# CEED/Laghos

Measured on AMD Instinct MI355X. Metric: Mdofs×steps/s on 3D Sedov -pa (Q3/Q2), higher is better.
Workload: dtype f64; 1 GPU; 3D Sedov -p 1 -m cube01_hex -rs 4 -ok 3 -ot 2 -pa (32^3 elements, E0/2^dim = 0.125); transport=none (one rank), elements=32768, h1_dofs=2738019, l2_dofs=884736, quad_points_per_element=216, rk_stages_executed=1300, ode=RK4, parallelism=elements1x1x1, zones_per_gpu=32x32x32

## Files before the change

laghos_amd/csrc/lgh_api.hip:

```cpp
#include <cstdarg>
#include <cstdlib>
#include <cmath>
#include <algorithm>
#include <limits>

#include "lgh_common.hpp"

#include <atomic>
#include <chrono>
#include <dlfcn.h>

namespace lgh
{

static thread_local char g_err[512] = "";
void set_error(const char *fmt, ...)
{
   va_list ap;
   va_start(ap, fmt);
   vsnprintf(g_err, sizeof(g_err), fmt, ap);
   va_end(ap);
}

__global__ void __launch_bounds__(256) vec_set_k(double *y, double a, long n)
{
   for (long i = blockIdx.x * (long)blockDim.x + threadIdx.x; i < n; i += (long)gridDim.x * blockDim.x) { y[i] = a; }
}
__global__ void __launch_bounds__(256)
vec_axpby_k(double *z, double a, const double *x, double b, const double *y, long n)
{
   for (long i = blockIdx.x * (long)blockDim.x + threadIdx.x; i < n; i += (long)gridDim.x * blockDim.x)
   {
      z[i] = fma(a, x[i], __dmul_rn(b, y[i]));
   }
}
__global__ void __launch_bounds__(256)
vec_axpby2_k(double2 *z, double a, const double2 *x, double b, const double2 *y, long n2)
{
   const long stride = (long)gridDim.x * blockDim.x;
   long i = blockIdx.x * (long)blockDim.x + threadIdx.x;
   for (; i + stride < n2; i += 2 * stride)
   {
      const double2 x0 = x[i], y0 = y[i], x1 = x[i + stride], y1 = y[i + stride];
      z[i] = make_double2(fma(a, x0.x, __dmul_rn(b, y0.x)), fma(a, x0.y, __dmul_rn(b, y0.y)));
      z[i + stride] = make_double2(fma(a, x1.x, __dmul_rn(b, y1.x)), fma(a, x1.y, __dmul_rn(b, y1.y)));
   }
   if (i < n2)
   {
      const double2 x0 = x[i], y0 = y[i];
      z[i] = make_double2(fma(a, x0.x, __dmul_rn(b, y0.x)), fma(a, x0.y, __dmul_rn(b, y0.y)));
   }
}
__global__ void __launch_bounds__(256)
vec_axpby_pair_k(double2 *z1, double a1, const double2 *x1, double b1, double2 *z2, double a2, const double2 *x2, double b2, const double2 *y, long n2)
{
   const long stride = (long)gridDim.x * blockDim.x;
   for (long i = blockIdx.x * (long)blockDim.x + threadIdx.x; i < n2; i += stride)
   {
      const double2 y0 = y[i], p = x1[i], q = x2[i];
// ... 28 lines not shown
   }
}
__global__ void set_double_k(double *p, double v) { *p = v; }
__global__ void __launch_bounds__(256) dt_est_set_k(double *p, double v)
{
   if (threadIdx.x == 0) { p[0] = v; }
   for (int s = threadIdx.x; s < kDtSlots; s += blockDim.x) { p[kDtSlotStride * (1 + s)] = __builtin_inf(); }
}
__global__ void __launch_bounds__(256) dt_est_fold_k(double *p, const int *err, double *host_out, const unsigned long long token)
{
   __shared__ double red[16];
   double m = __builtin_inf();
   for (int s = threadIdx.x; s < kDtSlots; s += blockDim.x)
   {
      m = fmin(m, p[kDtSlotStride * (1 + s)]);
      p[kDtSlotStride * (1 + s)] = __builtin_inf();
   }
   m = block_min(m, red);
   if (threadIdx.x == 0)
   {
      const double est = fmin(p[0], m);
      p[0] = est;
      host_out[0] = est;
      ((int *)(host_out + 1))[0] = *err;
      __threadfence_system();
      __hip_atomic_store((unsigned long long *)(host_out + 2), token, __ATOMIC_RELEASE, __HIP_MEMORY_SCOPE_SYSTEM);
   }
}

int vec_set(lgh_ctx *c, double *y, double a, long n)
{
   if (n <= 0) { return LGH_OK; }
   hipLaunchKernelGGL(vec_set_k, dim3(grid_for(n)), dim3(256), 0, c->stream, y, a, n);
   LGH_HIP_CHECK(hipGetLastError());
   return LGH_OK;
}
int vec_axpby(lgh_ctx *c, double *z, double a, const double *x, double b, const double *y, long n)
{
   if (n <= 0) { return LGH_OK; }
   if (n >= 4096 && (((uintptr_t)z | (uintptr_t)x | (uintptr_t)y) & 15u) == 0)
   {
      const long n2 = n / 2;
      hipLaunchKernelGGL(vec_axpby2_k, dim3(grid_for(n2)), dim3(256), 0, c->stream, (double2 *)z, a, (const double2 *)x, b,
                         (const double2 *)y, n2);
      if (n & 1) { hipLaunchKernelGGL(vec_axpby_k, dim3(1), dim3(64), 0, c->stream, z + 2 * n2, a, x + 2 * n2, b, y + 2 * n2, 1L); }
   }
   else { hipLaunchKernelGGL(vec_axpby_k, dim3(grid_for(n)), dim3(256), 0, c->stream, z, a, x, b, y, n); }
   LGH_HIP_CHECK(hipGetLastError());
   return LGH_OK;
}
int vec_axpby_pair(lgh_ctx *c, double *z1, double a1, const double *x1, double b1, double *z2, double a2, const double *x2, double b2,
                   const double *y, long n)
{
   if (n <= 0) { return LGH_OK; }
   if (n >= 4096 && (((uintptr_t)z1 | (uintptr_t)x1 | (uintptr_t)z2 | (uintptr_t)x2 | (uintptr_t)y) & 15u) == 0)
   {
      const long n2 = n / 2;
      hipLaunchKernelGGL(vec_axpby_pair_k, dim3(grid_for(n2)), dim3(256), 0, c->stream, (double2 *)z1, a1, (const double2 *)x1, b1, (double2 *)z2, a2,
                         (const double2 *)x2, b2, (const double2 *)y, n2);
      LGH_HIP_CHECK(hipGetLastError());
      if (n & 1)
      {
         hipLaunchKernelGGL(vec_axpby_k, dim3(1), dim3(64), 0, c->stream, z1 + 2 * n2, a1, x1 + 2 * n2, b1, y + 2 * n2, 1L);
         hipLaunchKernelGGL(vec_axpby_k, dim3(1), dim3(64), 0, c->stream, z2 + 2 * n2, a2, x2 + 2 * n2, b2, y + 2 * n2, 1L);
      }
      LGH_HIP_CHECK(hipGetLastError());
// ... 527 lines not shown
   LGH_CHECK_ARG(c && on);
   *on = (!c->stress_store && c->erhs_q && c->force_e_q && c->v_snap && !c->fused_forces_off && c->dim == 3) ? 0 : 1;
   return LGH_OK;
}
int lgh_qupdate_store_stress(lgh_ctx *c, int on)
{
   LGH_CHECK_ARG(c);
   if ((on != 0) != (c->stress_store != 0))
   {
      c->stress_store = on ? 1 : 0;
      invalidate_fused(c);
      c->stress_current = 0;
   }
   return LGH_OK;
}
int lgh_reset_quadrature_data(lgh_ctx *c)
{
   LGH_CHECK_ARG(c);
   invalidate_fused(c);
   return LGH_OK;
}
int lgh_fused_force_mult(lgh_ctx *c, double *y_h1)
{
   LGH_CHECK_ARG(c && y_h1);
   if (!(c->force_e_q && c->fused_f1_valid)) { set_error("lgh_fused_force_mult: no fused F.1 on hand"); return LGH_ERR_ARG; }
   int rc = h1_transpose_gather(c, c->dim, c->force_e_q, y_h1);
   if (rc == LGH_OK && c->multi != 0) { rc = halo_sum(c, y_h1, c->dim); }
   return rc;
}
int lgh_fused_force_mult_transpose(lgh_ctx *c, double *y_l2)
{
   LGH_CHECK_ARG(c && y_l2);
   if (!(c->erhs_q && c->fused_ftv_valid)) { set_error("lgh_fused_force_mult_transpose: no fused F^T v on hand"); return LGH_ERR_ARG; }
   LGH_HIP_CHECK(hipMemcpyAsync(y_l2, c->erhs_q, sizeof(double) * (size_t)c->L2V, hipMemcpyDeviceToDevice, c->stream));
   return LGH_OK;
}
int lgh_quadrature_generation(lgh_ctx *c, unsigned long *gen, int *f1_valid, int *ftv_valid)
{
   LGH_CHECK_ARG(c && gen && f1_valid && ftv_valid);
   *gen = c->qgen;
   *f1_valid = c->fused_f1_valid;
   *ftv_valid = c->fused_ftv_valid;
   return LGH_OK;
}
double *lgh_qdata_Jac0inv(lgh_ctx *c) { return c->Jac0inv; }
double *lgh_qdata_rho0DetJ0w(lgh_ctx *c) { return c->rho0DetJ0w; }
double *lgh_mass_D(lgh_ctx *c)
{
   c->mass_rank1 = -1;
   c->mass_gen++;
   return c->massD;
}
int lgh_mass_data_form(lgh_ctx *c, int *form)
{
   LGH_CHECK_ARG(c && form);
   if (c->dim == 1) { *form = 0; return LGH_OK; }
   const double *Dq, *Se;
   int dqs;
   int rc = mass_data(c, &Dq, &dqs, &Se);
   if (rc) { return rc; }
   *form = (c->mass_rank1 == 1) ? 1 : 0;
   return LGH_OK;
}
int lgh_mass_data_changed(lgh_ctx *c)
{
   LGH_CHECK_ARG(c);
   c->mass_rank1 = -1;
   c->mass_gen++;
// ... 252 lines not shown
         for (int cc = 0; cc < dim; cc++)
         {
            c->timers.c[0] += its[cc];
            if (h1_iters) { *h1_iters += its[cc]; }
         }
         c->cur_ess = dim - 1;
         return LGH_OK;
      }
      if (rc != LGH_ERR_UNSUPPORTED) { return rc; }
   }
   for (int cc = 0; cc < dim; cc++)
   {
      LGH_HIP_CHECK(hipMemcpyAsync(work_B, rhs_h1 + (size_t)cc * N, sizeof(double) * N,
                                   hipMemcpyDeviceToDevice, c->stream));
      rc = lgh_mass_set_essential_tdofs(c, cc);
      if (rc) { return rc; }
      rc = lgh_mass_eliminate_rhs(c, work_B);
      if (rc) { return rc; }
      int it = 0;
      timer_start(c);
      rc = cg_solve(c, LGH_SPACE_H1, work_B, dv + (size_t)cc * N, rel_tol, max_iter, &it, true);
      timer_stop(c, 0);
      if (rc) { return rc; }
      c->timers.c[0] += it;
      if (h1_iters) { *h1_iters += it; }
   }
   return LGH_OK;
}

int lgh_vec_set(lgh_ctx *c, double *y, double a, long n) { LGH_CHECK_ARG(c && y); return vec_set(c, y, a, n); }
int lgh_vec_copy(lgh_ctx *c, double *y, const double *x, long n)
{
   LGH_CHECK_ARG(c && y && x);
   LGH_HIP_CHECK(hipMemcpyAsync(y, x, sizeof(double) * n, hipMemcpyDeviceToDevice, c->stream));
   return LGH_OK;
}
int lgh_vec_axpby(lgh_ctx *c, double *z, double a, const double *x, double b, const double *y, long n)
{
   LGH_CHECK_ARG(c && z && x && y);
   return vec_axpby(c, z, a, x, b, y, n);
}
int lgh_vec_axpby_pair(lgh_ctx *c, double *z1, double a1, const double *x1, double b1, double *z2, double a2, const double *x2, double b2,
                       const double *y, long n)
{
   LGH_CHECK_ARG(c && z1 && x1 && z2 && x2 && y && n >= 0);
   {
      auto overlap = [n](const double *p, const double *q) { return p < q + n && q < p + n; };
      LGH_CHECK_ARG(!overlap(z1, z2) && !overlap(z1, x2) && !overlap(z1, y));
      LGH_CHECK_ARG(!overlap(z2, y) && !overlap(z2, x1) && (z2 == x2 || !overlap(z2, x2)) && (z1 == x1 || !overlap(z1, x1)));
   }
   return vec_axpby_pair(c, z1, a1, x1, b1, z2, a2, x2, b2, y, n);
}
int lgh_vec_dot(lgh_ctx *c, const double *x, const double *y, long n, double *result)
{
   LGH_CHECK_ARG(c && x && y && result);
   int rc = vec_dot(c, x, y, nullptr, n, c->scal + 1);
   if (rc) { return rc; }
   LGH_HIP_CHECK(hipMemcpyAsync(c->host_pinned + kPinDot, c->scal + 1, sizeof(double), hipMemcpyDeviceToHost, c->stream));
   LGH_HIP_CHECK(hipStreamSynchronize(c->stream));
   *result = c->host_pinned[kPinDot];
   return LGH_OK;
}

int lgh_set_velocity_source(lgh_ctx *c, const double *accel_h1)
{
   LGH_CHECK_ARG(c);
   if (accel_h1)
   {
// ... 213 lines not shown
```

laghos_amd/csrc/lgh_common.hpp:

```cpp
#pragma once
#include <hip/hip_runtime.h>

#include <algorithm>
#include <cstdint>
#include <cstdio>
#include <cstring>
#include <string>
#include <vector>

#include "../../include/laghos_hip.h"

namespace lgh
{

void set_error(const char *fmt, ...);

#define LGH_HIP_CHECK(expr)                                                              \
   do                                                                                    \
   {                                                                                     \
      hipError_t e_ = (expr);                                                            \
      if (e_ != hipSuccess)                                                              \
      {                                                                                  \
         lgh::set_error("HIP error %s at %s:%d: %s", hipGetErrorName(e_), __FILE__,      \
                        __LINE__, #expr);                                                \
// ... 147 lines not shown
   lgh::ScalarCg *l2run = nullptr;
   const double *accel_src;
   lgh::EnergySolve energy;
   long ls_stats[3] = {0, 0, 0};
   bool own_stream;

   double *B, *G, *Bl, *W, *gamma;
   int *h1map;
   int *t_off;
   int *t_idx;
   int *t_ell;
   int t_deg;
   uint8_t *essmask[3];
   int *ess[3];
   int ess_count[3];
   double *owner;
   int cur_ess;

   double *stressJinvT, *Jac0inv, *rho0DetJ0w, *massD, *diagV, *dinvV;
   double *Jac0inv_soa;
   double *Jac0inv_e;
   int jac0_compact;
   double *massS, *ones_ne;
   double *M1h = nullptr, *M1l = nullptr;
   double *w1d = nullptr;
   int mass_rank1;
   double *dt_est_dev;
   double *erhs_q;
   double *v_snap;
   double *force_e_q;
   int fused_ftv_valid, fused_f1_valid;
   unsigned long qgen;
   int *dev_flags;
   double *ones_l2;
   int stress_store;
   int stress_current;
   int fused_forces_off;
   double *XE;
   double *YE;
   double *cg_r, *cg_z, *cg_d0, *cg_d1, *cg_y;
   double *partials;
   int part_stride;
   unsigned int *tickets;
   lgh::CgScalars *cgs;
   double *scal;
   double *host_pinned;
   unsigned long long look_token;
   double *host_pinned_dev;

   void *vcg_s;
   double *vcg_vec, *vcg_partials;
   unsigned int *vcg_tickets;
   unsigned vcg_stride;
   int vcg_last;
   int vcg_grid;
   int b_h1_sym, b_l2_sym;
   int ncu;
   void *vcg_aux;

   lgh::Timers timers;
   lgh::KTime *ktime;
   int cg_last_iters[2][3];
   lgh::Comm *comm;
   int nranks, rank;
   int multi;
   unsigned long long *q_trace_dev;
// ... 243 lines not shown
int vcg_test_exact_sum(lgh_ctx *c, int mode, long n, int G, int E, const double *scale, const double *v, const long long *w_in,
                       long long *w_out, double *d_out, int *i_out);
int vcg_k1_form(lgh_ctx *c);
void comm_shared_nodes(const lgh_ctx *c, const uint8_t **hmask, const int **sh_node, int *n_shared);
int energy_overlap_poll(lgh_ctx *c);
int host_wait_token(lgh_ctx *c, volatile unsigned long long *word, unsigned long long token);
constexpr int kLsWord = 50;
constexpr int kLsWordsPerSet = 56;
struct LockstepWords { const long long *own; const long long *peers; int n_peers, before; };
bool l2_lockstep_possible(lgh_ctx *c);
int cg_l2_begin_lockstep(lgh_ctx *c, const double *b, double *x, double rel_tol, int max_iter);
int l2_lockstep_limit(lgh_ctx *c);
int l2_lockstep_apply(lgh_ctx *c, int it, const LockstepWords &prev, double *den_mirror);
int l2_lockstep_update(lgh_ctx *c, int it, const double *den_src, long long *word_out);
int l2_lockstep_fold(lgh_ctx *c, int it, const LockstepWords &last);
int cg_l2_end_lockstep(lgh_ctx *c, int *iters);
int comm_ranks_before(const lgh_ctx *c);
bool vcg_lockstep_ready(const lgh_ctx *c);
int cg_l2_begin(lgh_ctx *c, const double *b, double *x, double rel_tol, int max_iter);
int cg_l2_end(lgh_ctx *c, int *iters);
void cg_l2_free(lgh_ctx *c);
int cg_solve(lgh_ctx *c, int space, const double *b, double *x, double rel_tol, int max_iter,
             int *iters, bool x_is_zero);
int stress_on_hand(lgh_ctx *c, const char *who);
int qupdate(lgh_ctx *c, const double *S);
int setup_rho0detj0(lgh_ctx *c, const double *x0, const double *rho0_l2, const double *rho0_q,
                    double *volume);
int interp_energy(lgh_ctx *c, int which, const double *vec, double *result);
int tg_source_2d(lgh_ctx *c, const double *S, double *out);
int test_eig(lgh_ctx *c, int dim, int n, const double *A, double *lambda, double *vec);
int test_singular(lgh_ctx *c, int dim, int n, const double *A, double *sv);
int test_sqrt(lgh_ctx *c, int n, const double *x, double *y);
int vec_set(lgh_ctx *c, double *y, double a, long n);
int vec_axpby(lgh_ctx *c, double *z, double a, const double *x, double b, const double *y, long n);
int vec_axpby_pair(lgh_ctx *c, double *z1, double a1, const double *x1, double b1, double *z2, double a2, const double *x2, double b2,
                   const double *y, long n);
int vec_neg_inplace(lgh_ctx *c, double *y, long n);
int vec_zero_list(lgh_ctx *c, double *y, const int *list, int n);
int vec_dot(lgh_ctx *c, const double *x, const double *y, const double *w, long n, double *dev_out);
struct HaloNodeAlias { const int *nodes, *sh_node; };
int halo_sum(lgh_ctx *c, double *v, int ncomp, double *extra = nullptr, int nextra = 0, bool packed = false, const HaloNodeAlias *alias = nullptr);
void comm_node_lists(const lgh_ctx *c, const int **nodes, int *total, const int **sh_node, int *n_shared);
struct HaloPackTables
{
   const int *sh_off, *sh_src;
   const int *pos, *cnt;
   const int *base, *ncnt;
   double *sbuf;
   int n_nbr;
};
bool comm_pack_tables(const lgh_ctx *c, HaloPackTables *t);
bool halo_can_piggyback(const lgh_ctx *c);
bool comm_second_channel(const lgh_ctx *c);
int exchange_words(lgh_ctx *c, const long long *src, int nwords);
int comm_word_peers(lgh_ctx *c, int nwords, const long long **peers, int *n_peers);
int allreduce_dev_n(lgh_ctx *c, double *dev, long count, int op);
int allreduce_dev(lgh_ctx *c, double *dev, int count, int op, bool packed = false);

bool kernel_id_supported_1d(int kid);
int create_1d(const lgh_config *cfg, lgh_ctx *c);
int setup_1d(lgh_ctx *c, const double *x0, const double *rho0_l2, const double *rho0_q, double *volume);
int mass_changed_1d(lgh_ctx *c);
int force_mult_1d(lgh_ctx *c, const double *x_l2, double *y_h1);
int force_mult_t_1d(lgh_ctx *c, const double *v_h1, double *y_l2);
int mass_apply_1d(lgh_ctx *c, int space, const double *x, double *y, bool eliminate);
int l2_solve_local_1d(lgh_ctx *c, const double *b, double *x);
// ... 44 lines not shown
```

laghos_amd/csrc/lgh_energy.hip:

```cpp
#include <algorithm>

#include "lgh_common.hpp"

extern "C"
{

__global__ void __launch_bounds__(256) vec_differs_k(const double *__restrict__ a, const double *__restrict__ b, const long n, int *flag)
{
   const long stride = (long)gridDim.x * blockDim.x, t = (long)blockIdx.x * blockDim.x + threadIdx.x;
   bool diff = false;
   if (((((uintptr_t)a) | ((uintptr_t)b)) & 15u) == 0)
   {
      const longlong2 *a2 = (const longlong2 *)a, *b2 = (const longlong2 *)b;
      for (long i = t; i < n / 2; i += stride)
      {
         const longlong2 p = a2[i], q = b2[i];
         diff = diff || p.x != q.x || p.y != q.y;
      }
      if ((n & 1) && t == 0) { diff = diff || __double_as_longlong(a[n - 1]) != __double_as_longlong(b[n - 1]); }
   }
   else
   {
      for (long i = t; i < n; i += stride) { diff = diff || __double_as_longlong(a[i]) != __double_as_longlong(b[i]); }
   }
// ... 14 lines not shown
{
   if (*flag != 0) { return; }
   const long i = (long)blockIdx.x * blockDim.x + threadIdx.x;
   if (i < n) { y[i] = x[i]; }
}

}

namespace lgh
{

struct Stream2Scope
{
   lgh_ctx *c;
   explicit Stream2Scope(lgh_ctx *c_) : c(c_) { flip(1); }
   ~Stream2Scope() { flip(0); }
   Stream2Scope(const Stream2Scope &) = delete;
   Stream2Scope &operator=(const Stream2Scope &) = delete;

private:
   void flip(const int on)
   {
      std::swap(c->stream, c->stream2);
      c->on_stream2 = on;
   }
};

static int energy_rhs(lgh_ctx *c, const double *v_h1, double *e_rhs)
{
   RoctxRange range("SolveEnergy-ForcePA");
   if (c->erhs_q && c->fused_ftv_valid)
   {
      int *flag = c->dev_flags + (c->on_stream2 ? 2 : 0);
      LGH_HIP_CHECK(hipMemsetAsync(flag, 0, sizeof(int), c->stream));
      hipLaunchKernelGGL(vec_differs_k, dim3(grid_for((c->H1V + 1) / 2)), dim3(256), 0, c->stream, v_h1, c->v_snap, (long)c->H1V, flag);
      LGH_HIP_CHECK(hipGetLastError());
      if (c->stress_current)
      {
         const int rc = force_mult_t_L(c, c->stressJinvT, v_h1, e_rhs, flag);
         if (rc) { return rc; }
         hipLaunchKernelGGL(copy_unless_k, dim3(ceil_div(c->L2V, 256)), dim3(256), 0, c->stream, e_rhs, c->erhs_q, (long)c->L2V, flag);
      }
      else
      {
         hipLaunchKernelGGL(erhs_take_or_poison_k, dim3(ceil_div(c->L2V, 256)), dim3(256), 0, c->stream, e_rhs, c->erhs_q, (long)c->L2V, flag, c->dev_flags + 4);
      }
      LGH_HIP_CHECK(hipGetLastError());
      return LGH_OK;
   }
   return lgh_force_mult_transpose(c, v_h1, e_rhs);
}
static int energy_rhs_with_source(lgh_ctx *c, const double *v_h1, double *e_rhs, const double *e_source)
{
   timer_start(c);
   int rc = energy_rhs(c, v_h1, e_rhs);
   timer_stop(c, 2);
   if (rc == LGH_OK && e_source) { rc = vec_axpby(c, e_rhs, 1.0, e_rhs, 1.0, e_source, c->L2V); }
   return rc;
}
static void count_l2(lgh_ctx *c, const int it, int *l2_iters)
{
   const int counted = (it == 0) ? 1 : it;
   c->timers.c[1] += counted;
   if (l2_iters) { *l2_iters += counted; }
}

static int create_stream2(lgh_ctx *c)
// ... 159 lines not shown
```

laghos_amd/csrc/lgh_qupdate.hip:

```cpp
#include "lgh_qpoint.hpp"
#include "lgh_qrows.hpp"

namespace lgh
{

int qupdate_form(lgh_ctx *c);
int qupdate(lgh_ctx *c, const double *S)
{
   QArgs a = q_base(c);
   a.x = S;
   a.v = S + c->H1V;
   a.e = S + 2 * (size_t)c->H1V;
   a.result = c->dt_est_dev;
   a.Jac0inv_e = (c->jac0_compact == 1) ? c->Jac0inv_e : nullptr;
   const bool keep = !c->stress_store && a.erhs_q && a.force_e && c->v_snap;
   if (keep) { a.stressJinvT = nullptr; }
   const int form = qupdate_form(c);
   const int rc = (form == 1) ? launch_qrows(c, a) : launch_q<QMODE_UPDATE>(c, a);
   c->qgen++;
   c->stress_current = (rc == LGH_OK && !keep) ? 1 : 0;
   c->fused_ftv_valid = (rc == LGH_OK && a.erhs_q && c->v_snap) ? 1 : 0;
   c->fused_f1_valid = (rc == LGH_OK && a.force_e) ? 1 : 0;
   if (c->fused_ftv_valid)
   {
      LGH_HIP_CHECK(hipMemcpyAsync(c->v_snap, S + c->H1V, sizeof(double) * (size_t)c->H1V, hipMemcpyDeviceToDevice, c->stream));
   }
   return rc;
}

int qupdate_form(lgh_ctx *c)
{
   return (qrows_available(c) && c->sw.q_form) ? 1 : 0;
}

int interp_energy(lgh_ctx *c, int which, const double *vec, double *result)
{
   QArgs a = q_base(c);
   a.result = c->scal;
   int rc;
   if (which == 0)
   {
      a.e = vec;
      rc = launch_q<QMODE_IE>(c, a);
   }
   else
   {
      a.v = vec;
      rc = launch_q<QMODE_KE>(c, a);
   }
   if (rc) { return rc; }
   if (c->multi != 0)
   {
      rc = allreduce_dev(c, c->scal, 1, 0);
      if (rc) { return rc; }
   }
   LGH_HIP_CHECK(hipMemcpyAsync(c->host_pinned + kPinResult, c->scal, sizeof(double), hipMemcpyDeviceToHost, c->stream));
   LGH_HIP_CHECK(hipStreamSynchronize(c->stream));
   *result = (which == 0) ? c->host_pinned[kPinResult] : 0.5 * c->host_pinned[kPinResult];
// ... 111 lines not shown
```

laghos_amd/csrc/lgh_vcg.hip:

```cpp
#include "lgh_vcg.hpp"

namespace lgh
{
typedef unsigned v4u_ __attribute__((ext_vector_type(4)));

__device__ __forceinline__ double vcg_ld(const double *base, const unsigned off) { return *(const double *)((const char *)base + off); }
__device__ __forceinline__ double *vcg_ptr(double *base, const unsigned off) { return (double *)((char *)base + off); }

__device__ __forceinline__ void vcg_reset_accumulators(const VcgArgs &a)
{
   if (!a.reset || blockIdx.x != 0) { return; }
   if (a.limbs) { for (int i = threadIdx.x; i < 2 * kLimbWords + 8 * 16; i += blockDim.x) { a.limbs[i] = 0; } }
   if (a.rzl) { for (int i = threadIdx.x; i < 3 * kLimbWords; i += blockDim.x) { a.rzl[i] = 0; } }
}
__device__ __forceinline__ void vcg_reset_scalars(const VcgArgs &a, VcgScalars *s)
{
   if (!a.reset) { return; }
   s->rel_tol2 = a.reset_tol2;
   s->all_done = 0;
   s->first = 1;
   for (int c = 0; c < kVC; c++) { s->done[c] = 0; s->iters[c] = 0; s->nupd[c] = 0; s->alpha_last[c] = 0.0; s->alpha_hist[0][c] = s->alpha_hist[1][c] = 0.0; s->rzh[0][c] = s->rzh[1][c] = 0.0; }
}

__global__ void __launch_bounds__(256)
// ... 67 lines not shown
#pragma unroll
         for (int j = 0; j < DEG; j++) { if (pos[j] >= 0) { s += FE[pos[j] + (long)ND * c]; } }
         double bv = -s;
         if (a.ess[c] && a.ess[c][n]) { bv = 0.0; }
         const size_t i = (size_t)c * a.N + n;
         bout[(size_t)c * a.N + (a.ncaller ? a.ncaller[n] : n)] = bv;
         a.r[i] = bv;
         a.x[i] = 0.0;
         part[c] = __dmul_rn(bv, di) * bv;
      }
   }
   double bp[kVC], total[kVC];
   block_sum3(part[0], part[1], part[2], red, bp);
   if (grid_sum3_last_block(bp, a.partials, a.stride, a.ticket, red, total))
   {
      if (threadIdx.x == 0)
      {
         VcgScalars *s = a.s;
         int all = 1;
         vcg_reset_scalars(a, s);
         for (int c = 0; c < kVC; c++)
         {
            s->rz[c] = s->rz_prev[c] = total[c];
            s->iters[c] = 0;
            s->r0[c] = fmax(total[c] * s->rel_tol2, 0.0);
            s->done[c] = (total[c] < 0.0 || total[c] <= s->r0[c]) ? 1 : 0;
            all = all && s->done[c];
         }
         s->first = 1;
         s->all_done = all;
      }
   }
}
__global__ void __launch_bounds__(256)
vcg_init_force_z_k(const VcgArgs a, const double *__restrict__ FE, const unsigned compb_fe, const unsigned *__restrict__ ellf,
                   double *__restrict__ bout)
{
   vcg_reset_accumulators(a);
   __shared__ double red[48];
   const int n = xcd_swizzle(blockIdx.x, gridDim.x) * blockDim.x + threadIdx.x;
   const bool ok = n < a.N;
   const unsigned nn = (unsigned)(ok ? n : a.N - 1);
   const unsigned rowb = 4u * (unsigned)a.N;
   unsigned ix[8];
#pragma unroll
   for (int j = 0; j < 8; j++) { ix[j] = *(const unsigned *)((const char *)ellf + (4u * nn + (unsigned)j * rowb)); }
   const double di = vcg_ld(a.dinv, 8u * nn);
   const unsigned es = a.essbits[nn];
   const unsigned zoff = 8u * (unsigned)kVC * (unsigned)(a.ye_stride - kYePad);
   double fe[kVC][8];
#pragma unroll
   for (int j = 0; j < 8; j++)
   {
      if (j == 0 || __any(ix[j] != zoff))
      {
#pragma unroll
         for (int c = 0; c < kVC; c++) { fe[c][j] = vcg_ld(FE, ix[j] + (unsigned)c * compb_fe); }
      }
      else
      {
#pragma unroll
         for (int c = 0; c < kVC; c++) { fe[c][j] = 0.0; }
      }
   }
   double part[kVC];
#pragma unroll
   for (int c = 0; c < kVC; c++)
   {
      double s = 0.0;
#pragma unroll
      for (int j = 0; j < 8; j++) { s += fe[c][j]; }
      double bv = -s;
      if ((es >> c) & 1u) { bv = 0.0; }
      part[c] = ok ? __dmul_rn(bv, di) * bv : 0.0;
      if (ok)
      {
         const size_t i = (size_t)c * a.N + n;
         bout[(size_t)c * a.N + (a.ncaller ? a.ncaller[n] : n)] = bv;
         a.r[i] = bv;
         a.x[i] = 0.0;
      }
   }
   double bp[kVC], total[kVC];
   block_sum3(part[0], part[1], part[2], red, bp);
   if (grid_sum3_last_block(bp, a.partials, a.stride, a.ticket, red, total))
   {
      if (threadIdx.x == 0)
      {
         VcgScalars *s = a.s;
         int all = 1;
         vcg_reset_scalars(a, s);
         for (int c = 0; c < kVC; c++)
         {
            s->rz[c] = s->rz_prev[c] = total[c];
            s->iters[c] = 0;
            s->r0[c] = fmax(total[c] * s->rel_tol2, 0.0);
            s->done[c] = (total[c] < 0.0 || total[c] <= s->r0[c]) ? 1 : 0;
            all = all && s->done[c];
         }
         s->first = 1;
         s->all_done = all;
      }
   }
}
__global__ void vcg_init_finish_k(VcgScalars *s)
{
   int all = 1;
   for (int c = 0; c < kVC; c++)
   {
      s->rz_prev[c] = s->rz[c];
      s->r0[c] = fmax(s->rz[c] * s->rel_tol2, 0.0);
      s->done[c] = (s->rz[c] < 0.0 || s->rz[c] <= s->r0[c]) ? 1 : 0;
      all = all && s->done[c];
// ... 184 lines not shown
   }
   if (a.rzl && !(todo[0] || todo[1] || todo[2]))
   {
      if (blockIdx.x == 0 && tid == 0)
      {
         for (int k = 0; k < kVC; k++) { if (!a.s->done[k] && den[k] == 0.0) { a.s->done[k] = 1; } }
      }
      return;
   }
   const bool xload = XU && it > 2;
   const unsigned compb = 8u * (unsigned)a.N;
   const unsigned zoff = 8u * (unsigned)(a.ye_stride - kYePad);
   const char *const ellhi = (const char *)a.ellz + (size_t)16 * (size_t)a.N;
   double part[kVC] = {0.0, 0.0, 0.0};
   for (int base = n0; base < n1; base += NT)
   {
      const int n = base + tid;
      const bool ok = n < n1;
      const unsigned nn = (unsigned)(ok ? n : n0);
      unsigned ix[4];
      const v4u_ q0 = *(const v4u_ *)((const char *)a.ellz + 16u * nn);
      ix[0] = q0[0]; ix[1] = q0[1]; ix[2] = q0[2]; ix[3] = q0[3];
      const bool hi = !a.k2_skip || __any(q0[3] != zoff);
      double ro[kVC], dol[kVC], xo[kVC];
      const double di = vcg_ld(a.dinv, 8u * nn);
      const unsigned es = a.essbits[nn];
#pragma unroll
      for (int k = 0; k < kVC; k++)
      {
         const unsigned vb = 8u * nn + (unsigned)k * compb;
         ro[k] = vcg_ld(a.r, vb);
         dol[k] = vcg_ld(a.d, vb);
         xo[k] = 0.0;
         if (XU && MINW < 6) { xo[k] = vcg_ld(a.x, vb); }
      }
      bool need[4];
      need[0] = true;
#pragma unroll
      for (int j = 1; j < 4; j++) { need[j] = !a.k2_skip || __any(ix[j] != zoff); }
      double zsum[kVC];
      {
         double ye[kVC][4];
#pragma unroll
         for (int j = 0; j < 4; j++)
         {
            if (need[j])
            {
#pragma unroll
               for (int k = 0; k < kVC; k++) { ye[k][j] = vcg_ld(a.YE + (size_t)k * a.ye_stride, ix[j]); }
            }
            else
            {
#pragma unroll
               for (int k = 0; k < kVC; k++) { ye[k][j] = 0.0; }
            }
         }
#pragma unroll
         for (int k = 0; k < kVC; k++) { zsum[k] = ((0.0 + ye[k][0]) + ye[k][1]) + ye[k][2]; zsum[k] += ye[k][3]; }
      }
      if (XU && MINW >= 6 && xload)
      {
#pragma unroll
         for (int k = 0; k < kVC; k++) { asm volatile("" : "+v"(zsum[k])); xo[k] = vcg_ld(a.x, 8u * nn + (unsigned)k * compb); }
      }
      if (hi)
      {
         const v4u_ q1 = *(const v4u_ *)(ellhi + 16u * nn);
// ... 87 lines not shown
         for (int k = 0; k < kVC; k++)
         {
            if (a.den_limbs == 1 && !s->done[k])
            {
               s->den[k] = den[k];
               if (den[k] == 0.0) { s->done[k] = 1; }
            }
            if (!s->done[k] && !(a.multi && s->den[k] == 0.0))
            {
               s->alpha_last[k] = s->rz[k] / den[k];
               s->nupd[k] = it;
               s->rz_prev[k] = s->rz[k];
               s->rz[k] = total[k];
               if (!a.multi)
               {
                  s->iters[k] = it;
                  if (total[k] < 0.0 || total[k] <= s->r0[k]) { s->done[k] = 1; }
               }
            }
            all = all && s->done[k];
         }
         if (!a.multi) { s->all_done = all; }
         if (a.pack_rz)
         {
            for (int k = 0; k < a.hp.n_nbr; k++)
            {
               for (int e = 0; e < kVC; e++) { a.hp.sbuf[(size_t)a.hp.base[k] + e] = s->rz[e]; }
            }
         }
      }
   }
}
__global__ void __launch_bounds__(256)
vcg_xfix_k(const VcgArgs a)
{
   const int n = blockIdx.x * blockDim.x + threadIdx.x;
   if (n >= a.N) { return; }
   for (int k = 0; k < kVC; k++)
   {
      if ((a.s->nupd[k] & 1) == 0) { continue; }
      const size_t i = (size_t)k * a.N + n;
      a.x[i] = fma(a.s->alpha_last[k], a.d[i], a.x[i]);
   }
}

__global__ void __launch_bounds__(256)
vcg_xout_k(const VcgArgs a, double *__restrict__ X)
{
   const int n = blockIdx.x * blockDim.x + threadIdx.x;
   if (n >= a.N) { return; }
   const int nc = a.ncaller[n];
   for (int k = 0; k < kVC; k++)
   {
      const size_t i = (size_t)k * a.N + n;
      double xv = a.x[i];
      if (a.s->nupd[k] & 1) { xv = fma(a.s->alpha_last[k], a.d[i], xv); }
      X[(size_t)k * a.N + nc] = xv;
   }
}

__global__ void __launch_bounds__(256)
vcg_gather_k(const VcgArgs a)
{
   const int n = blockIdx.x * blockDim.x + threadIdx.x;
   if (n >= a.N) { return; }
   for (int c = 0; c < kVC; c++)
   {
      if (a.s->done[c]) { continue; }
      const double *yc = a.YE + (size_t)c * a.ye_stride;
      double s = 0.0;
      for (int j = 0; j < a.deg; j++)
      {
         const int p = a.ell[(size_t)j * a.N + n];
         if (p >= 0) { s += yc[p]; }
      }
// ... 247 lines not shown
   if (m.pack_halo) { (void)comm_pack_tables(c, &a.hp); }
   a.pack_halo = m.pack_halo;
   a.nx_den = m.nx_den;
   a.pack_rz = m.pack_rz;
   return LGH_OK;
}

int vcg_prepare(lgh_ctx *c, double *B, double *X, double rel_tol, VcgPlan &plan, const bool in_solve)
{
   LGH_VCG_TRY(vcg_work_buffers(c));
   if (!c->vcg_aux) { LGH_VCG_TRY(vcg_build_aux(c)); }
   VcgAux *aux = (VcgAux *)c->vcg_aux;
   plan.aux = aux;
   plan.k1 = vcg_resolve_k1(c);
   LGH_VCG_TRY(vcg_mode(c, aux, plan.k1, in_solve, plan.mode));
   const VcgMode &m = plan.mode;
   if (!in_solve)
   {
      hipLaunchKernelGGL(vcg_set_tol_k, dim3(1), dim3(1), 0, c->stream, (VcgScalars *)c->vcg_s, rel_tol * rel_tol, m.limbs ? aux->limbs.p : nullptr,
                         m.rzl ? aux->rzl.p : nullptr);
   }
   return vcg_fill_args(c, aux, plan.k1, m, B, X, rel_tol, in_solve, plan.a);
}

static_assert((kPinVcg + (sizeof(VcgScalars) + sizeof(double) - 1) / sizeof(double)) <= (size_t)kPinVcgToken, "VcgScalars ends before the token slot of the pinned block");

struct VcgRun
{
   VcgScalars *ds, *hs;
   const HaloNodeAlias *alias;
   int max_iter, chunk, it = 0, looks = 0;
   bool energy_polled = false;
   int ls_limit, ls_before;
};

static int vcg_start(lgh_ctx *c, VcgPlan &plan, double *B, const double *force_E)
{
   VcgArgs &a = plan.a;
   const VcgAux *aux = plan.aux;
   const int nb = ceil_div(a.N, 256);
   a.partials = c->vcg_partials;
   a.ticket = c->vcg_tickets;
   if (force_E)
   {
      if (!plan.mode.direct) { set_error("vcg_solve: fused init is single-rank, degree <= 8"); return LGH_ERR_ARG; }
      if (aux->ellf && aux->essbits) { hipLaunchKernelGGL(vcg_init_force_z_k, dim3(nb), dim3(256), 0, c->stream, a, force_E, 8u * (unsigned)c->ND, aux->ellf, B); }
      else { hipLaunchKernelGGL(vcg_init_force_k<8>, dim3(nb), dim3(256), 0, c->stream, a, force_E, c->ND, B, aux->o_ellc ? aux->o_ellc : c->t_ell, c->t_deg); }
   }
   else
   {
      if (aux->ord) { LGH_HIP_CHECK(hipMemsetAsync(a.x, 0, kVC * (size_t)a.N * sizeof(double), c->stream)); }
      hipLaunchKernelGGL(vcg_init_k, dim3(nb), dim3(256), 0, c->stream, a);
   }
   LGH_HIP_CHECK(hipGetLastError());
   if (plan.mode.multi)
   {
      LGH_VCG_TRY(allreduce_dev(c, a.s->rz, kVC, 0));
      hipLaunchKernelGGL(vcg_init_finish_k, dim3(1), dim3(1), 0, c->stream, a.s);
   }
   return LGH_OK;
}

static int vcg_look(lgh_ctx *c, const VcgPlan &plan, VcgRun &r, bool &stop)
{
   const VcgArgs &a = plan.a;
   VcgScalars *hs_dev = (VcgScalars *)(c->host_pinned_dev + kPinVcg);
   unsigned long long *tok_dev = (unsigned long long *)(c->host_pinned_dev + kPinVcgToken);
   volatile unsigned long long *tok = (volatile unsigned long long *)(c->host_pinned + kPinVcgToken);
   const unsigned long long token = ++c->look_token;
   bool copied = false;
   if (!r.energy_polled) { r.energy_polled = true; LGH_VCG_TRY(energy_overlap_poll(c)); }
   if (plan.mode.multi && !a.rzl && r.it > 0) { hipLaunchKernelGGL(vcg_update_finish_k, dim3(1), dim3(1), 0, c->stream, r.ds, r.it, hs_dev, tok_dev, token); copied = true; }
   if (a.rzl && r.it > 0) { vcg_launch_rz_finish(c, a, r.it, hs_dev, tok_dev, token); copied = true; }
   if (copied)
   {
      LGH_VCG_TRY(host_wait_token(c, tok, token));
   }
   else
   {
      LGH_HIP_CHECK(hipMemcpyAsync(r.hs, r.ds, sizeof(VcgScalars), hipMemcpyDeviceToHost, c->stream));
      LGH_HIP_CHECK(hipStreamSynchronize(c->stream));
   }
   stop = r.hs->all_done || r.it >= r.max_iter;
   if (!stop) { r.chunk = (++r.looks <= 2) ? 2 : std::min(64, 2 * r.chunk); }
   return LGH_OK;
}

static int vcg_step_k1(lgh_ctx *c, const VcgPlan &plan, VcgArgs &a)
{
   a.partials = c->vcg_partials + (size_t)kVC * c->vcg_stride;
   a.ticket = c->vcg_tickets + kTicketSlot;
   kt_begin(c, LGH_KERNEL_MASS_CG_H1);
   vcg_launch_k1(c, plan, a);
   kt_end(c, LGH_KERNEL_MASS_CG_H1);
   LGH_HIP_CHECK(hipGetLastError());
   a.partials = c->vcg_partials;
   a.ticket = c->vcg_tickets;
   return LGH_OK;
}

static int vcg_iterate_direct(lgh_ctx *c, const VcgPlan &plan, VcgArgs &a)
{
   LGH_VCG_TRY(vcg_step_k1(c, plan, a));
   if (plan.mode.k2p) { vcg_launch_k2p(c, plan, a, a.iter); }
   else { kt_begin(c, LGH_KERNEL_CG_UPDATE_H1); vcg_launch_update(c, a, true); kt_end(c, LGH_KERNEL_CG_UPDATE_H1); }
   LGH_HIP_CHECK(hipGetLastError());
   return LGH_OK;
}

static int vcg_iterate_exchange(lgh_ctx *c, const VcgPlan &plan, VcgArgs &a, const VcgRun &r, const int upto)
{
   const VcgMode &m = plan.mode;
   const int it = a.iter, nb = ceil_div(a.N, 256);
   const bool ls_it = m.ls && it <= r.ls_limit;
   auto ls_words = [&](const int set_it) { return LockstepWords{a.rzl + (set_it % 3) * kLimbWords, a.rzl_peers, a.n_rz_peers, r.ls_before}; };
   LGH_VCG_TRY(vcg_step_k1(c, plan, a));
// ... 10 lines not shown
   }
   LGH_HIP_CHECK(hipGetLastError());
   if (m.multi)
   {
      const bool ride = halo_can_piggyback(c);
      LGH_VCG_TRY(halo_sum(c, a.yL, kVC, ride ? r.ds->den : nullptr, ride ? std::max(a.nx_den, kVC) : 0, a.pack_halo != 0, r.alias));
      if (!ride) { LGH_VCG_TRY(allreduce_dev(c, r.ds->den, kVC, 0)); }
   }
   if (m.mixed && m.k2p) { vcg_launch_k2p(c, plan, a, it); }
   else { vcg_launch_update(c, a, m.mixed); }
   if (ls_it) { LGH_VCG_TRY(l2_lockstep_update(c, it, &r.ds->den_e, a.rzl + (it % 3) * kLimbWords)); }
   if (m.multi && a.rzl)
   {
      LGH_VCG_TRY(exchange_words(c, a.rzl + (it % 3) * kLimbWords, kLimbWords));
      if (ls_it && (it == r.ls_limit || it == upto))
      {
         LGH_VCG_TRY(l2_lockstep_fold(c, it, ls_words(it)));
      }
   }
   else if (m.multi) { LGH_VCG_TRY(allreduce_dev(c, r.ds->rz, kVC, 0, a.pack_rz != 0 && m.mixed && m.k2p)); }
   LGH_HIP_CHECK(hipGetLastError());
   return LGH_OK;
}

static int vcg_finish(lgh_ctx *c, const VcgPlan &plan, const VcgRun &r, double *X, int iters[3])
{
   const VcgArgs &a = plan.a;
   const int nb = ceil_div(a.N, 256);
   if (plan.aux->ord)
   {
      hipLaunchKernelGGL(vcg_xout_k, dim3(nb), dim3(256), 0, c->stream, a, X);
      LGH_HIP_CHECK(hipGetLastError());
   }
   else if (plan.mode.k2p && ((r.hs->nupd[0] | r.hs->nupd[1] | r.hs->nupd[2]) & 1))
   {
      hipLaunchKernelGGL(vcg_xfix_k, dim3(nb), dim3(256), 0, c->stream, a);
      LGH_HIP_CHECK(hipGetLastError());
   }
   FILE *f = a.trace ? fopen(c->sw.vcg_trace.c_str(), "w") : nullptr;
   if (f)
   {
      std::vector<unsigned long long> h((size_t)kTraceRec * kTraceBlocks);
      (void)hipMemcpy(h.data(), a.trace, h.size() * 8, hipMemcpyDeviceToHost);
      for (int i = 0; i < kTraceBlocks; i++)
      {
         if (h[(size_t)kTraceRec * i] == 0) { continue; }
         fprintf(f, "%d", i);
         for (int k = 0; k < kTraceRec; k++) { fprintf(f, " %llu", h[(size_t)kTraceRec * i + k]); }
         fprintf(f, "\n");
      }
      fclose(f);
   }
   int mx = 0;
   for (int k = 0; k < kVC; k++)
   {
      int fin = r.hs->iters[k];
      if (!r.hs->done[k] && r.it >= r.max_iter) { fin = r.max_iter; }
      iters[k] = fin;
      mx = std::max(mx, fin);
   }
   c->vcg_last = mx;
   return LGH_OK;
}

int vcg_solve(lgh_ctx *c, double *B, double *X, double rel_tol, int max_iter, int iters[3], const double *force_E)
{
   if (!vcg_available(c)) { return LGH_ERR_UNSUPPORTED; }
   VcgPlan plan;
   LGH_VCG_TRY(vcg_prepare(c, B, X, rel_tol, plan, true));
   VcgArgs &a = plan.a;
   const VcgMode &m = plan.mode;
   VcgRun r;
   r.ds = a.s;
   r.hs = (VcgScalars *)(c->host_pinned + kPinVcg);
   r.alias = (plan.aux->ord && plan.aux->o_alias.nodes) ? &plan.aux->o_alias : nullptr;
   r.max_iter = max_iter;
   r.chunk = c->vcg_last > 0 ? c->vcg_last : 8;
   r.ls_limit = m.ls ? std::min(l2_lockstep_limit(c), max_iter) : 0;
   r.ls_before = m.ls ? comm_ranks_before(c) : 0;
   LGH_VCG_TRY(vcg_start(c, plan, B, force_E));
   for (bool first_look = true;; first_look = false)
   {
      if (!first_look || max_iter <= 0)
      {
         bool stop = false;
         LGH_VCG_TRY(vcg_look(c, plan, r, stop));
         if (stop) { break; }
      }
      const int upto = std::min(max_iter, r.it + r.chunk);
      while (r.it < upto)
      {
         a.iter = ++r.it;
         LGH_VCG_TRY(m.direct ? vcg_iterate_direct(c, plan, a) : vcg_iterate_exchange(c, plan, a, r, upto));
      }
   }
   return vcg_finish(c, plan, r, X, iters);
}

}
```

laghos_amd/csrc/lgh_vcg_tables.hip:

```cpp
#include <memory>
#include "lgh_vcg.hpp"

namespace lgh
{

__global__ void __launch_bounds__(256)
vcg_ellf_k(const int *__restrict__ ell, unsigned *__restrict__ ellf, const size_t n_have, const size_t n_all, const int ND, const int NE)
{
   const size_t i = (size_t)blockIdx.x * blockDim.x + threadIdx.x;
   if (i >= n_all) { return; }
   const int p = (i < n_have) ? ell[i] : -1;
   const int e = p / ND;
   ellf[i] = 8u * (unsigned)(p < 0 ? kVC * ND * NE : kVC * ND * e + (p - e * ND));
}
__global__ void __launch_bounds__(256)
vcg_mapb_k(const int *__restrict__ map, unsigned *__restrict__ mapb, const size_t n)
{
   const size_t i = (size_t)blockIdx.x * blockDim.x + threadIdx.x;
   if (i < n) { mapb[i] = 8u * (unsigned)map[i]; }
}
__global__ void __launch_bounds__(256)
vcg_map_xrows_k(const int *__restrict__ map, const size_t nrows, const int D, int *flag)
{
   const size_t i = (size_t)blockIdx.x * blockDim.x + threadIdx.x;
   if (i >= nrows) { return; }
   const int *p = map + i * D;
   bool ok = true;
   for (int k = 1; k < D; k++) { ok = ok && p[k] == p[0] + k; }
   if (!ok) { *flag = 1; }
}
__global__ void __launch_bounds__(256)
vcg_essbits_k(const uint8_t *e0, const uint8_t *e1, const uint8_t *e2, const uint8_t *hmask, const double *owner, uint8_t *bits,
              const int N)
{
   const int n = blockIdx.x * blockDim.x + threadIdx.x;
   if (n >= N) { return; }
   bits[n] = (uint8_t)(((e0 && e0[n]) ? 1 : 0) | ((e1 && e1[n]) ? 2 : 0) | ((e2 && e2[n]) ? 4 : 0) | ((hmask && hmask[n]) ? 8 : 0) |
                       ((owner && owner[n] == 0.0) ? 16 : 0));
}
__global__ void __launch_bounds__(256)
vcg_ellz_k(const int *__restrict__ ell, unsigned *__restrict__ ellz, const size_t n_have, const size_t n_all, const int zslot)
{
   const size_t i = (size_t)blockIdx.x * blockDim.x + threadIdx.x;
   if (i >= n_all) { return; }
   const int p = (i < n_have) ? ell[i] : -1;
   const size_t N = n_all / 8, j = i / N, n = i - j * N;
// ... 266 lines not shown
```

Baseline: 1612 Mdofs*steps/s.

## Fuse flag clears into copy kernel, skip x zeroing, interleave ellf table

Device-to-device memcpy calls become a custom vectorized copy kernel. The snapshot copy also clears the energy-difference flags, which removes the separate memset launches that followed it. The force-init kernel no longer zeroes x; that work moves into a gated xfix kernel launched early during the convergence look, and the iteration skips loading x. The ellf table is laid out as two interleaved 4-wide blocks so one vector load fetches four indices and the upper half is read only when needed. Together these cut launches and memory traffic, at the cost of more complex state tracking across solve phases.

```diff
diff --git a/laghos_amd/csrc/lgh_api.hip b/laghos_amd/csrc/lgh_api.hip
--- a/laghos_amd/csrc/lgh_api.hip
+++ b/laghos_amd/csrc/lgh_api.hip
@@ -25,6 +25,35 @@
 __global__ void __launch_bounds__(256) vec_set_k(double *y, double a, long n)
 {
    for (long i = blockIdx.x * (long)blockDim.x + threadIdx.x; i < n; i += (long)gridDim.x * blockDim.x) { y[i] = a; }
+}
+__global__ void __launch_bounds__(256)
+vec_copy_k(long long *y, const long long *x, const long n, int *clear0, int *clear1)
+{
+   const long stride = (long)gridDim.x * blockDim.x, t = blockIdx.x * (long)blockDim.x + threadIdx.x;
+   if (t == 0)
+   {
+      if (clear0) { *clear0 = 0; }
+      if (clear1) { *clear1 = 0; }
+   }
+   if (((((uintptr_t)y) | ((uintptr_t)x)) & 15u) == 0)
+   {
+      longlong2 *y2 = (longlong2 *)y;
+      const longlong2 *x2 = (const longlong2 *)x;
+      const long n2 = n / 2;
+      long i = t;
+      for (; i + stride < n2; i += 2 * stride)
+      {
+         const longlong2 p = x2[i], q = x2[i + stride];
+         y2[i] = p;
+         y2[i + stride] = q;
+      }
+      if (i < n2) { y2[i] = x2[i]; }
+      if ((n & 1) && t == 0) { y[n - 1] = x[n - 1]; }
+   }
+   else
+   {
+      for (long i = t; i < n; i += stride) { y[i] = x[i]; }
+   }
 }
 __global__ void __launch_bounds__(256)
 vec_axpby_k(double *z, double a, const double *x, double b, const double *y, long n)
@@ -119,6 +148,14 @@
 {
    if (n <= 0) { return LGH_OK; }
    hipLaunchKernelGGL(vec_set_k, dim3(grid_for(n)), dim3(256), 0, c->stream, y, a, n);
+   LGH_HIP_CHECK(hipGetLastError());
+   return LGH_OK;
+}
+int vec_copy(lgh_ctx *c, double *y, const double *x, long n, int *clear0, int *clear1)
+{
+   if (n <= 0 && !clear0 && !clear1) { return LGH_OK; }
+   n = std::max<long>(n, 0);
+   hipLaunchKernelGGL(vec_copy_k, dim3(grid_for((n + 1) / 2)), dim3(256), 0, c->stream, (long long *)y, (const long long *)x, n, clear0, clear1);
    LGH_HIP_CHECK(hipGetLastError());
    return LGH_OK;
 }
@@ -712,8 +749,7 @@
 {
    LGH_CHECK_ARG(c && y_l2);
    if (!(c->erhs_q && c->fused_ftv_valid)) { set_error("lgh_fused_force_mult_transpose: no fused F^T v on hand"); return LGH_ERR_ARG; }
-   LGH_HIP_CHECK(hipMemcpyAsync(y_l2, c->erhs_q, sizeof(double) * (size_t)c->L2V, hipMemcpyDeviceToDevice, c->stream));
-   return LGH_OK;
+   return vec_copy(c, y_l2, c->erhs_q, c->L2V);
 }
 int lgh_quadrature_generation(lgh_ctx *c, unsigned long *gen, int *f1_valid, int *ftv_valid)
 {
@@ -1032,8 +1068,7 @@
 int lgh_vec_copy(lgh_ctx *c, double *y, const double *x, long n)
 {
    LGH_CHECK_ARG(c && y && x);
-   LGH_HIP_CHECK(hipMemcpyAsync(y, x, sizeof(double) * n, hipMemcpyDeviceToDevice, c->stream));
-   return LGH_OK;
+   return vec_copy(c, y, x, n);
 }
 int lgh_vec_axpby(lgh_ctx *c, double *z, double a, const double *x, double b, const double *y, long n)
 {
diff --git a/laghos_amd/csrc/lgh_common.hpp b/laghos_amd/csrc/lgh_common.hpp
--- a/laghos_amd/csrc/lgh_common.hpp
+++ b/laghos_amd/csrc/lgh_common.hpp
@@ -203,6 +203,7 @@
    int fused_ftv_valid, fused_f1_valid;
    unsigned long qgen;
    int *dev_flags;
+   int vdiff_clear;
    double *ones_l2;
    int stress_store;
    int stress_current;
@@ -512,6 +513,7 @@
 int test_singular(lgh_ctx *c, int dim, int n, const double *A, double *sv);
 int test_sqrt(lgh_ctx *c, int n, const double *x, double *y);
 int vec_set(lgh_ctx *c, double *y, double a, long n);
+int vec_copy(lgh_ctx *c, double *y, const double *x, long n, int *clear0 = nullptr, int *clear1 = nullptr);
 int vec_axpby(lgh_ctx *c, double *z, double a, const double *x, double b, const double *y, long n);
 int vec_axpby_pair(lgh_ctx *c, double *z1, double a1, const double *x1, double b1, double *z2, double a2, const double *x2, double b2,
                    const double *y, long n);
diff --git a/laghos_amd/csrc/lgh_energy.hip b/laghos_amd/csrc/lgh_energy.hip
--- a/laghos_amd/csrc/lgh_energy.hip
+++ b/laghos_amd/csrc/lgh_energy.hip
@@ -70,7 +70,9 @@
    if (c->erhs_q && c->fused_ftv_valid)
    {
       int *flag = c->dev_flags + (c->on_stream2 ? 2 : 0);
-      LGH_HIP_CHECK(hipMemsetAsync(flag, 0, sizeof(int), c->stream));
+      const int bit = c->on_stream2 ? 2 : 1;
+      if (c->vdiff_clear & bit) { c->vdiff_clear &= ~bit; }
+      else { LGH_HIP_CHECK(hipMemsetAsync(flag, 0, sizeof(int), c->stream)); }
       hipLaunchKernelGGL(vec_differs_k, dim3(grid_for((c->H1V + 1) / 2)), dim3(256), 0, c->stream, v_h1, c->v_snap, (long)c->H1V, flag);
       LGH_HIP_CHECK(hipGetLastError());
       if (c->stress_current)
diff --git a/laghos_amd/csrc/lgh_qupdate.hip b/laghos_amd/csrc/lgh_qupdate.hip
--- a/laghos_amd/csrc/lgh_qupdate.hip
+++ b/laghos_amd/csrc/lgh_qupdate.hip
@@ -23,7 +23,10 @@
    c->fused_f1_valid = (rc == LGH_OK && a.force_e) ? 1 : 0;
    if (c->fused_ftv_valid)
    {
-      LGH_HIP_CHECK(hipMemcpyAsync(c->v_snap, S + c->H1V, sizeof(double) * (size_t)c->H1V, hipMemcpyDeviceToDevice, c->stream));
+      c->vdiff_clear = 0;
+      const int rcs = vec_copy(c, c->v_snap, S + c->H1V, c->H1V, c->dev_flags + 0, c->dev_flags + 2);
+      if (rcs) { return rcs; }
+      c->vdiff_clear = 3;
    }
    return rc;
 }
diff --git a/laghos_amd/csrc/lgh_vcg.hip b/laghos_amd/csrc/lgh_vcg.hip
--- a/laghos_amd/csrc/lgh_vcg.hip
+++ b/laghos_amd/csrc/lgh_vcg.hip
@@ -123,6 +123,7 @@
       }
    }
 }
+template <bool ZX>
 __global__ void __launch_bounds__(256)
 vcg_init_force_z_k(const VcgArgs a, const double *__restrict__ FE, const unsigned compb_fe, const unsigned *__restrict__ ellf,
                    double *__restrict__ bout)
@@ -132,21 +133,25 @@
    const int n = xcd_swizzle(blockIdx.x, gridDim.x) * blockDim.x + threadIdx.x;
    const bool ok = n < a.N;
    const unsigned nn = (unsigned)(ok ? n : a.N - 1);
-   const unsigned rowb = 4u * (unsigned)a.N;
-   unsigned ix[8];
-#pragma unroll
-   for (int j = 0; j < 8; j++) { ix[j] = *(const unsigned *)((const char *)ellf + (4u * nn + (unsigned)j * rowb)); }
+   const unsigned zoff = 8u * (unsigned)kVC * (unsigned)(a.ye_stride - kYePad);
+   const v4u_ q0 = *(const v4u_ *)((const char *)ellf + 16u * nn);
    const double di = vcg_ld(a.dinv, 8u * nn);
    const unsigned es = a.essbits[nn];
-   const unsigned zoff = 8u * (unsigned)kVC * (unsigned)(a.ye_stride - kYePad);
+   const bool hi = __any(q0[3] != zoff);
+   v4u_ q1 = {zoff, zoff, zoff, zoff};
+   if (hi) { q1 = *(const v4u_ *)((const char *)ellf + (size_t)16 * (size_t)a.N + 16u * nn); }
+   bool need[4];
+   need[0] = true;
+#pragma unroll
+   for (int j = 1; j < 4; j++) { need[j] = __any(q0[j] != zoff); }
    double fe[kVC][8];
 #pragma unroll
-   for (int j = 0; j < 8; j++)
-   {
-      if (j == 0 || __any(ix[j] != zoff))
-      {
-#pragma unroll
-         for (int c = 0; c < kVC; c++) { fe[c][j] = vcg_ld(FE, ix[j] + (unsigned)c * compb_fe); }
+   for (int j = 0; j < 4; j++)
+   {
+      if (need[j])
+      {
+#pragma unroll
+         for (int c = 0; c < kVC; c++) { fe[c][j] = vcg_ld(FE, q0[j] + (unsigned)c * compb_fe); }
       }
       else
       {
@@ -154,13 +159,21 @@
          for (int c = 0; c < kVC; c++) { fe[c][j] = 0.0; }
       }
    }
+   if (hi)
+   {
+#pragma unroll
+      for (int j = 0; j < 4; j++)
+      {
+#pragma unroll
+         for (int c = 0; c < kVC; c++) { fe[c][4 + j] = vcg_ld(FE, q1[j] + (unsigned)c * compb_fe); }
+      }
+   }
    double part[kVC];
 #pragma unroll
    for (int c = 0; c < kVC; c++)
    {
-      double s = 0.0;
-#pragma unroll
-      for (int j = 0; j < 8; j++) { s += fe[c][j]; }
+      double s = (((0.0 + fe[c][0]) + fe[c][1]) + fe[c][2]) + fe[c][3];
+      if (hi) { s = (((s + fe[c][4]) + fe[c][5]) + fe[c][6]) + fe[c][7]; }
       double bv = -s;
       if ((es >> c) & 1u) { bv = 0.0; }
       part[c] = ok ? __dmul_rn(bv, di) * bv : 0.0;
@@ -169,7 +182,7 @@
          const size_t i = (size_t)c * a.N + n;
          bout[(size_t)c * a.N + (a.ncaller ? a.ncaller[n] : n)] = bv;
          a.r[i] = bv;
-         a.x[i] = 0.0;
+         if (ZX) { a.x[i] = 0.0; }
       }
    }
    double bp[kVC], total[kVC];
@@ -420,7 +433,7 @@
          ro[k] = vcg_ld(a.r, vb);
          dol[k] = vcg_ld(a.d, vb);
          xo[k] = 0.0;
-         if (XU && MINW < 6) { xo[k] = vcg_ld(a.x, vb); }
+         if (XU && MINW < 6 && xload) { xo[k] = vcg_ld(a.x, vb); }
       }
       bool need[4];
       need[0] = true;
@@ -574,15 +587,23 @@
    }
 }
 __global__ void __launch_bounds__(256)
-vcg_xfix_k(const VcgArgs a)
-{
+vcg_xfix_k(const VcgArgs a, const int xz, const int gated, const int at_limit)
+{
+   if (gated && !(a.s->all_done || at_limit)) { return; }
    const int n = blockIdx.x * blockDim.x + threadIdx.x;
    if (n >= a.N) { return; }
    for (int k = 0; k < kVC; k++)
    {
-      if ((a.s->nupd[k] & 1) == 0) { continue; }
+      const int nu = a.s->nupd[k];
       const size_t i = (size_t)k * a.N + n;
-      a.x[i] = fma(a.s->alpha_last[k], a.d[i], a.x[i]);
+      if (nu == 0)
+      {
+         if (xz) { a.x[i] = 0.0; }
+         continue;
+      }
+      if ((nu & 1) == 0) { continue; }
+      const double x0 = (xz && nu == 1) ? 0.0 : a.x[i];
+      a.x[i] = fma(a.s->alpha_last[k], a.d[i], x0);
    }
 }
 
@@ -896,9 +917,12 @@
    int max_iter, chunk, it = 0, looks = 0;
    bool energy_polled = false;
    int ls_limit, ls_before;
+   bool xz = false;
+   bool xfix_ahead = false;
+   bool xfixed = false;
 };
 
-static int vcg_start(lgh_ctx *c, VcgPlan &plan, double *B, const double *force_E)
+static int vcg_start(lgh_ctx *c, VcgPlan &plan, VcgRun &r, double *B, const double *force_E)
 {
    VcgArgs &a = plan.a;
    const VcgAux *aux = plan.aux;
@@ -908,7 +932,9 @@
    if (force_E)
    {
       if (!plan.mode.direct) { set_error("vcg_solve: fused init is single-rank, degree <= 8"); return LGH_ERR_ARG; }
-      if (aux->ellf && aux->essbits) { hipLaunchKernelGGL(vcg_init_force_z_k, dim3(nb), dim3(256), 0, c->stream, a, force_E, 8u * (unsigned)c->ND, aux->ellf, B); }
+      r.xz = aux->ellf && aux->essbits && plan.mode.k2p && !aux->ord;
+      if (r.xz) { hipLaunchKernelGGL(vcg_init_force_z_k<false>, dim3(nb), dim3(256), 0, c->stream, a, force_E, 8u * (unsigned)c->ND, aux->ellf, B); }
+      else if (aux->ellf && aux->essbits) { hipLaunchKernelGGL(vcg_init_force_z_k<true>, dim3(nb), dim3(256), 0, c->stream, a, force_E, 8u * (unsigned)c->ND, aux->ellf, B); }
       else { hipLaunchKernelGGL(vcg_init_force_k<8>, dim3(nb), dim3(256), 0, c->stream, a, force_E, c->ND, B, aux->o_ellc ? aux->o_ellc : c->t_ell, c->t_deg); }
    }
    else
@@ -936,6 +962,8 @@
    if (!r.energy_polled) { r.energy_polled = true; LGH_VCG_TRY(energy_overlap_poll(c)); }
    if (plan.mode.multi && !a.rzl && r.it > 0) { hipLaunchKernelGGL(vcg_update_finish_k, dim3(1), dim3(1), 0, c->stream, r.ds, r.it, hs_dev, tok_dev, token); copied = true; }
    if (a.rzl && r.it > 0) { vcg_launch_rz_finish(c, a, r.it, hs_dev, tok_dev, token); copied = true; }
+   const bool ahead = copied && r.xfix_ahead;
+   if (ahead) { hipLaunchKernelGGL(vcg_xfix_k, dim3(ceil_div(a.N, 256)), dim3(256), 0, c->stream, a, r.xz ? 1 : 0, 1, r.it >= r.max_iter ? 1 : 0); }
    if (copied)
    {
       LGH_VCG_TRY(host_wait_token(c, tok, token));
@@ -946,6 +974,7 @@
       LGH_HIP_CHECK(hipStreamSynchronize(c->stream));
    }
    stop = r.hs->all_done || r.it >= r.max_iter;
+   r.xfixed = stop && ahead;
    if (!stop) { r.chunk = (++r.looks <= 2) ? 2 : std::min(64, 2 * r.chunk); }
    return LGH_OK;
 }
@@ -1022,9 +1051,11 @@
       hipLaunchKernelGGL(vcg_xout_k, dim3(nb), dim3(256), 0, c->stream, a, X);
       LGH_HIP_CHECK(hipGetLastError());
    }
-   else if (plan.mode.k2p && ((r.hs->nupd[0] | r.hs->nupd[1] | r.hs->nupd[2]) & 1))
-   {
-      hipLaunchKernelGGL(vcg_xfix_k, dim3(nb), dim3(256), 0, c->stream, a);
+   else if (plan.mode.k2p && !r.xfixed)
+   {
+      bool need = false;
+      for (int k = 0; k < kVC; k++) { need = need || (r.hs->nupd[k] & 1) || (r.xz && r.hs->nupd[k] == 0); }
+      if (need) { hipLaunchKernelGGL(vcg_xfix_k, dim3(nb), dim3(256), 0, c->stream, a, r.xz ? 1 : 0, 0, 0); }
       LGH_HIP_CHECK(hipGetLastError());
    }
    FILE *f = a.trace ? fopen(c->sw.vcg_trace.c_str(), "w") : nullptr;
@@ -1068,7 +1099,8 @@
    r.chunk = c->vcg_last > 0 ? c->vcg_last : 8;
    r.ls_limit = m.ls ? std::min(l2_lockstep_limit(c), max_iter) : 0;
    r.ls_before = m.ls ? comm_ranks_before(c) : 0;
-   LGH_VCG_TRY(vcg_start(c, plan, B, force_E));
+   LGH_VCG_TRY(vcg_start(c, plan, r, B, force_E));
+   r.xfix_ahead = m.direct && m.k2p && !plan.aux->ord;
    for (bool first_look = true;; first_look = false)
    {
       if (!first_look || max_iter <= 0)
diff --git a/laghos_amd/csrc/lgh_vcg_tables.hip b/laghos_amd/csrc/lgh_vcg_tables.hip
--- a/laghos_amd/csrc/lgh_vcg_tables.hip
+++ b/laghos_amd/csrc/lgh_vcg_tables.hip
@@ -11,7 +11,8 @@
    if (i >= n_all) { return; }
    const int p = (i < n_have) ? ell[i] : -1;
    const int e = p / ND;
-   ellf[i] = 8u * (unsigned)(p < 0 ? kVC * ND * NE : kVC * ND * e + (p - e * ND));
+   const size_t N = n_all / 8, j = i / N, n = i - j * N;
+   ellf[(j < 4 ? 0 : 4 * N) + 4 * n + (j & 3)] = 8u * (unsigned)(p < 0 ? kVC * ND * NE : kVC * ND * e + (p - e * ND));
 }
 __global__ void __launch_bounds__(256)
 vcg_mapb_k(const int *__restrict__ map, unsigned *__restrict__ mapb, const size_t n)
```

Measured after the change: 1627 Mdofs*steps/s, median of 6. About the same (+0.9%).
